# luo-yining/CFDBench

Hardware: NVIDIA H100
Metric: fno_rollout_steps_per_sec (higher is better)
Workload: dtype bf16

## Files before the change

### cfdbench_b200/_lib.py

```python
from __future__ import annotations

import ctypes as C
import os

_HERE = os.path.dirname(os.path.abspath(__file__))
LIB_PATH = os.path.join(_HERE, "libcfdbench_b200.so")

FNO_MAX_LAYERS = 8
ABI_VERSION = 4
ACT_F32, ACT_BF16 = 0, 1
EPI_GELU, EPI_GELU_SAVE_PRE, EPI_MUL_DGELU, EPI_PLAIN = 0, 1, 2, 3


class FnoWeights(C.Structure):
    _fields_ = [
        ("n_layers", C.c_int32),
        ("n_case_params", C.c_int32),
        ("fc0_w", C.c_void_p),
        ("fc0_b", C.c_void_p),
        ("spec_wk", C.c_void_p * FNO_MAX_LAYERS),
        ("w0t", C.c_void_p * FNO_MAX_LAYERS),
        ("w0_b", C.c_void_p * FNO_MAX_LAYERS),
        ("fc1_w", C.c_void_p),
        ("fc1_b", C.c_void_p),
# ... 28 lines not shown
    _fields_ = [("act", C.c_void_p * (FNO_MAX_LAYERS + 1)), ("pre", C.c_void_p * FNO_MAX_LAYERS),
                ("xm", C.c_void_p * FNO_MAX_LAYERS)]


class FnoWeightsBwd(C.Structure):
    _fields_ = [("spec_wkT", C.c_void_p * FNO_MAX_LAYERS), ("w0", C.c_void_p * FNO_MAX_LAYERS)]


class FnoBwdScratch(C.Structure):
    _fields_ = [("d", C.c_void_p * 2), ("dz1", C.c_void_p), ("gm", C.c_void_p), ("gwk", C.c_void_p),
                ("partials", C.c_void_p)]


BWD_CHUNK = 32
ADAM_MAX_TENSORS = 32


class FnoAdamTensors(C.Structure):
    _fields_ = [("count", C.c_int32),
                ("param", C.c_void_p * ADAM_MAX_TENSORS), ("grad", C.c_void_p * ADAM_MAX_TENSORS),
                ("exp_avg", C.c_void_p * ADAM_MAX_TENSORS), ("exp_avg_sq", C.c_void_p * ADAM_MAX_TENSORS),
                ("n", C.c_int64 * ADAM_MAX_TENSORS)]


class FnoNoise(C.Structure):
    _fields_ = [("std", C.c_float), ("seed", C.c_uint64), ("idx", C.c_void_p), ("step_base", C.c_void_p),
                ("step_offset", C.c_void_p), ("k0", C.c_int32)]


NOISE_STREAMS = 2 ** 16

_P = C.c_void_p
_I = C.c_int
_F = C.c_float

SIGNATURES = {
    "fno_version": (C.c_int, []),
    "fno_last_error": (C.c_char_p, []),
    "fno_destroy": (C.c_int, []),
    "fno_act_bytes": (C.c_size_t, [_I, _I]),
    "fno_modes_bytes": (C.c_size_t, [_I]),
    "fno_z_bytes": (C.c_size_t, [_I]),
    "fno_ym_image_bytes": (C.c_size_t, [_I]),
    "fno_bwd_partials_bytes": (C.c_size_t, []),
    "fno_mode_mix_image": (C.c_int, [_P, _P, _P, _I, _P]),
    "fno_block_fused": (C.c_int, [_P, _P, _P, _P, _P, _I, _P]),
    "fno_pack_spectral_weights": (C.c_int, [_P, _P, _P, _I, _P]),
    "fno_unpack_spectral_grads": (C.c_int, [_P, _P, _P, _P]),
    "fno_mix_operand_bytes": (C.c_size_t, []),
    "fno_pack_mix_operand": (C.c_int, [_P, _P, _P]),
    "fno_pack_mix_operand_from_weights": (C.c_int, [_P, _P, _P, _I, _P]),
    "fno_lift_fwd": (C.c_int, [_P, _P, _P, C.POINTER(FnoWeights), _P, _I, _I, _P]),
    "fno_spectral_dft_fwd": (C.c_int, [_P, _P, _I, _I, _F, _F, _P]),
    "fno_mode_mix": (C.c_int, [_P, _P, _P, _I, _P]),
    "fno_spectral_inv_kx": (C.c_int, [_P, _P, _I, _F, _F, _P]),
    "fno_block_out": (C.c_int, [_I, _P, _P, _P, _P, _P, _P, _P, _I, _I, _P]),
    "fno_block_fwd": (C.c_int, [C.POINTER(FnoWeights), _I, _P, _P, _P, C.POINTER(FnoWorkspace), _I, _I, _P]),
    "fno_project_fwd": (C.c_int, [_P, _P, C.POINTER(FnoWeights), _P, _I, _I, _P]),
    "fno_forward": (C.c_int, [C.POINTER(FnoWeights), _P, _P, _P, _P, C.POINTER(FnoWorkspace), _I, _I, _P]),
    "fno_rollout": (C.c_int, [C.POINTER(FnoWeights), _P, _P, _P, _P, _I, C.POINTER(FnoWorkspace), _I, _I, _P]),
    "fno_rollout_host": (C.c_int, [C.POINTER(FnoWeights), _P, _P, _P, _P, _I, C.POINTER(FnoWorkspace), _P, _I, _I, _P]),
    "fno_rollout_host_scratch_bytes": (C.c_size_t, [_I, _I, _I]),
    "fno_multistep_metrics": (C.c_int, [_P, _P, _P, _P, _I, _I, _P]),
    "fno_gather_batch": (C.c_int, [_P, _P, _P, _P, _P, _I, _I, _I, _P, _P, _P, _P, _P]),
    "fno_loss_scratch_bytes": (C.c_size_t, []),
    "fno_loss_fwd": (C.c_int, [_P, _P, C.c_size_t, _P, _P, _P]),
    "fno_loss_bwd": (C.c_int, [_P, _P, _P, _P, _P, C.c_size_t, _P]),
    "fno_adam_step": (C.c_int, [C.POINTER(FnoAdamTensors), C.c_float, C.c_float, C.c_float, C.c_float, C.c_float,
                                C.c_int64, _P]),
    "fno_train_stage_indices": (C.c_int, [_P, C.c_int64, _I, _I, _P, _P, _P]),
    "fno_adam_step_dev": (C.c_int, [C.POINTER(FnoAdamTensors), _P, _I, _P, _F, _F, _F, _F, _P]),
    "fno_adam_coefficients": (C.c_int, [_F, _F, _F, C.c_int64, _I, _P]),
    "fno_train_log_step": (C.c_int, [_P, _P, _I, _P, _P]),
    "fno_forward_train": (C.c_int, [C.POINTER(FnoWeights), _P, _P, _P, _P, C.POINTER(FnoTrainSaved),
                                    C.POINTER(FnoWorkspace), _I, _I, _P]),
    "fno_backward": (C.c_int, [C.POINTER(FnoWeights), C.POINTER(FnoWeightsBwd), _P, _P, _P, _P,
                               C.POINTER(FnoTrainSaved), C.POINTER(FnoGrads), C.POINTER(FnoBwdScratch),
                               C.POINTER(FnoWorkspace), _I, _I, _P]),
    "fno_backward_inputs": (C.c_int, [C.POINTER(FnoWeights), C.POINTER(FnoWeightsBwd), _P, _P, _P, _P,
                                      C.POINTER(FnoTrainSaved), C.POINTER(FnoGrads), C.POINTER(FnoBwdScratch),
                                      C.POINTER(FnoWorkspace), _P, _P, _I, _I, _P]),
    "fno_rollout_forward_train": (C.c_int, [C.POINTER(FnoWeights), _P, _P, _P, _P, _I, C.POINTER(FnoTrainSaved),
                                            C.POINTER(FnoWorkspace), _I, _I, _P]),
    "fno_rollout_backward": (C.c_int, [C.POINTER(FnoWeights), C.POINTER(FnoWeightsBwd), _P, _P, _P, _P, _P, _I,
                                       C.POINTER(FnoTrainSaved), C.POINTER(FnoGrads), C.POINTER(FnoBwdScratch),
                                       C.POINTER(FnoWorkspace), _P, _P, _P, _I, _I, _P]),
    "fno_grid_act_bytes": (C.c_size_t, [_I, _I, _I]),
    "fno_grid_z_bytes": (C.c_size_t, [_I, _I]),
    "fno_grid_bwd_partials_bytes": (C.c_size_t, [_I, _I]),
    "fno_grid_lift_fwd": (C.c_int, [_P, _P, _P, C.POINTER(FnoWeights), _P, _I, _I, _I, _P]),
    "fno_grid_spectral_dft_fwd": (C.c_int, [_P, _P, _I, _I, _I, _F, _F, _P]),
    "fno_grid_spectral_inv_kx": (C.c_int, [_P, _P, _I, _I, _I, _F, _F, _P]),
    "fno_grid_block_out": (C.c_int, [_I, _P, _P, _P, _P, _P, _P, _P, _I, _I, _I, _P]),
    "fno_grid_project_fwd": (C.c_int, [_P, _P, C.POINTER(FnoWeights), _P, _I, _I, _I, _P]),
    "fno_grid_project_bwd": (C.c_int, [_P, _P, _P, _P, C.POINTER(FnoWeights), _P, _P, _P, _P, _P, _P, _P, _I, _I, _I, _P]),
    "fno_grid_forward": (C.c_int, [C.POINTER(FnoWeights), _P, _P, _P, _P, C.POINTER(FnoWorkspace), _I, _I, _I, _P]),
    "fno_grid_rollout": (C.c_int, [C.POINTER(FnoWeights), _P, _P, _P, _P, _I, C.POINTER(FnoWorkspace), _I, _I, _I, _P]),
    "fno_grid_forward_train": (C.c_int, [C.POINTER(FnoWeights), _P, _P, _P, _P, C.POINTER(FnoTrainSaved),
                                         C.POINTER(FnoWorkspace), _I, _I, _I, _P]),
    "fno_grid_backward": (C.c_int, [C.POINTER(FnoWeights), C.POINTER(FnoWeightsBwd), _P, _P, _P, _P,
                                    C.POINTER(FnoTrainSaved), C.POINTER(FnoGrads), C.POINTER(FnoBwdScratch),
                                    C.POINTER(FnoWorkspace), _P, _P, _I, _I, _I, _P]),
    "fno_grid_rollout_forward_train": (C.c_int, [C.POINTER(FnoWeights), _P, _P, _P, _P, _I, C.POINTER(FnoTrainSaved),
                                                 C.POINTER(FnoWorkspace), _I, _I, _I, _P]),
    "fno_grid_rollout_backward": (C.c_int, [C.POINTER(FnoWeights), C.POINTER(FnoWeightsBwd), _P, _P, _P, _P, _P, _I,
                                            C.POINTER(FnoTrainSaved), C.POINTER(FnoGrads), C.POINTER(FnoBwdScratch),
# ... 65 lines not shown
```

### cfdbench_b200/csrc/fno_abi.cu

```cuda
#include <stdio.h>
#include <string.h>

#include "../../include/cfdbench_b200.h"
#include "fno_common.cuh"

namespace fno {
cudaError_t launch_dft_fwd(const void*, void*, int, float, float, cudaStream_t);
cudaError_t launch_mode_mix(const void*, const void*, void*, void*, int, cudaStream_t);
cudaError_t launch_block_fused(const void*, const void*, const float*, const float*, void*, int, cudaStream_t);
size_t ym_image_bytes(int);
cudaError_t launch_pack_spectral(const void*, const void*, void*, int, cudaStream_t);
cudaError_t launch_unpack_spectral(const void*, void*, void*, int, cudaStream_t);
cudaError_t launch_dft_fwd_tc(const void*, void*, int, float, float, cudaStream_t);
cudaError_t launch_pack_mix_operand(const void*, void*, cudaStream_t);
cudaError_t launch_pack_mix_operand_direct(const void*, const void*, void*, int, cudaStream_t);
size_t mix_operand_bytes();
cudaError_t launch_gather_batch(const void*, const void*, const float*, const int*, const long long*, int, int, int, float*,
                                float*, float*, float*, cudaStream_t);
cudaError_t launch_loss_fwd(const float*, const float*, size_t, float*, float*, cudaStream_t);
cudaError_t launch_loss_bwd(const float*, const float*, const float*, const float*, float*, size_t, cudaStream_t);
size_t loss_scratch_bytes();
cudaError_t launch_adam_step(const fno_adam_tensors*, float, float, float, float, float, long long, cudaStream_t);
cudaError_t launch_adam_step_dev(const fno_adam_tensors*, const float*, int, const int*, float, float, float, float,
                                 cudaStream_t);
void adam_coefficients(float, float, float, long long, float*, float*);
cudaError_t launch_stage_indices(const long long*, long long, int, int, const int*, long long*, cudaStream_t);
cudaError_t launch_log_step(const float*, float*, int, int*, cudaStream_t);
cudaError_t launch_inv_kx(const void*, void*, int, float, float, cudaStream_t);
template <typename TAct>
cudaError_t launch_block_tc(int, const void*, const void*, const float*, const float*, void*, float*, const float*, int,
                            cudaStream_t);
template <typename TAct>
cudaError_t launch_lift(const float*, const float*, const float*, const float*, const float*, const float*,
                        const float*, void*, int, int, cudaStream_t);
template <typename TAct>
cudaError_t launch_project_tc(const void*, const float*, const float*, const float*, const float*, const float*,
                              float*, int, cudaStream_t);
int project_bwd_rows_max();
int project_bwd_row();
cudaError_t launch_reduce_partials(const float*, int, int, float*, int, float*, int, float*, int, int, cudaStream_t);
template <typename TAct>
cudaError_t launch_project_bwd_tc(const void*, const float*, const float*, const float*, const float*, const float*, const float*,
                                  float*, float*, float*, int*, int, cudaStream_t);
template <typename TP, typename TQ, int NJ, int NI>
cudaError_t launch_chan_outer(const void*, const void*, float*, int*, int, cudaStream_t);
cudaError_t launch_multistep_metrics(const float*, const float*, const float*, float*, int, int, cudaStream_t);
cudaError_t launch_spectral_wgrad(const void*, const void*, void*, int, cudaStream_t);
cudaError_t launch_lift_bwd(const float*, const float*, const float*, const float*, const float*, const float*,
                            float*, float*, float*, int, int, int, cudaStream_t);
cudaError_t launch_lift_bwd_data(const float*, const float*, float*, float*, const float*, int, int, int, cudaStream_t);
bool grid_ok(int, int);
void grid_tables_release(int);
cudaError_t launch_grid_lift(const float*, const float*, const float*, const float*, const float*, const float*,
                             const float*, float*, int, int, int, int, cudaStream_t);
cudaError_t launch_grid_dft(const float*, void*, int, int, int, float, float, cudaStream_t);
cudaError_t launch_grid_inv_kx(const void*, float*, int, int, int, float, float, cudaStream_t);
cudaError_t launch_grid_block_out(int, const float*, const float*, const float*, const float*, float*, float*, const float*,
                                  int, int, int, cudaStream_t);
cudaError_t launch_grid_project(const float*, const float*, const float*, const float*, const float*, const float*, float*,
                                int, int, cudaStream_t);
cudaError_t launch_grid_project_bwd(const float*, const float*, const float*, const float*, const float*, const float*,
                                    const float*, float*, float*, float*, int, int, cudaStream_t);
int grid_project_bwd_parts(int, int);
int grid_project_bwd_row();
template <int NJ, int NI>
cudaError_t launch_grid_chan_outer(const float*, const float*, float*, int*, int, int, cudaStream_t);
// ... 135 lines not shown
const char* fno_last_error(void) { return g_err; }

size_t fno_act_bytes(int batch, int act_dtype) {
  return static_cast<size_t>(batch) * kC * kHW * (act_dtype == FNO_ACT_BF16 ? 2 : 4);
}
size_t fno_modes_bytes(int batch) { return static_cast<size_t>(batch) * kModes * kC * sizeof(float2); }
size_t fno_z_bytes(int batch) { return static_cast<size_t>(batch) * kH * 2 * kM2 * kC * sizeof(float); }
size_t fno_ym_image_bytes(int batch) { return ym_image_bytes(batch); }
size_t fno_bwd_partials_bytes(void) {
  return (static_cast<size_t>(296) * (kProj * kC + kProj) + static_cast<size_t>(project_bwd_rows_max()) * project_bwd_row() +
          static_cast<size_t>(16) * kC * (5 + kMaxCaseParams + 1)) * sizeof(float);
}

int fno_pack_spectral_weights(const void* w1, const void* w2, void* wk, int conj_transpose, void* stream) {
  if (!w1 || !w2 || !wk) return fail(kErrArg, "fno_pack_spectral_weights: null pointer");
  FNO_CUDA(launch_pack_spectral(w1, w2, wk, conj_transpose, S(stream)), "pack_spectral_kernel");
  return kOk;
}

size_t fno_mix_operand_bytes(void) { return mix_operand_bytes(); }

int fno_pack_mix_operand(const void* wk, void* wop, void* stream) {
  if (!wk || !wop) return fail(kErrArg, "fno_pack_mix_operand: null pointer");
  FNO_CUDA(launch_pack_mix_operand(wk, wop, S(stream)), "pack_mix_operand_kernel");
  return kOk;
}

int fno_pack_mix_operand_from_weights(const void* w1, const void* w2, void* wop, int conj_transpose, void* stream) {
  if (!w1 || !w2 || !wop) return fail(kErrArg, "fno_pack_mix_operand_from_weights: null pointer");
  FNO_CUDA(launch_pack_mix_operand_direct(w1, w2, wop, conj_transpose, S(stream)), "pack_mix_operand_direct_kernel");
  return kOk;
}

int fno_unpack_spectral_grads(const void* gwk, void* gw1, void* gw2, void* stream) {
  if (!gwk || !gw1 || !gw2) return fail(kErrArg, "fno_unpack_spectral_grads: null pointer");
  FNO_CUDA(launch_unpack_spectral(gwk, gw1, gw2, 0, S(stream)), "unpack_spectral_kernel");
  return kOk;
}

int fno_lift_fwd(const float* inputs, const float* mask, const float* case_params, const fno_weights* w,
                 void* act_out, int batch, int act_dtype, void* stream) {
  if (!inputs || !mask || !w || !act_out || batch <= 0 || bad_dtype(act_dtype))
    return fail(kErrArg, "fno_lift_fwd: bad argument");
  if (w->n_case_params > 0 && !case_params) return fail(kErrArg, "fno_lift_fwd: case_params is null");
  cudaError_t e = act_dtype == FNO_ACT_F32
                      ? launch_lift<float>(inputs, mask, case_params, w->fc0_w, w->fc0_b, w->gx, w->gy, act_out, batch,
                                           w->n_case_params, S(stream))
                      : launch_lift<__nv_bfloat16>(inputs, mask, case_params, w->fc0_w, w->fc0_b, w->gx, w->gy,
                                                   act_out, batch, w->n_case_params, S(stream));
  FNO_CUDA(e, "lift_kernel");
  return kOk;
}

int fno_spectral_dft_fwd(const void* act_in, void* xm, int batch, int act_dtype, float s0, float s1, void* stream) {
  if (!act_in || !xm || batch <= 0 || bad_dtype(act_dtype)) return fail(kErrArg, "fno_spectral_dft_fwd: bad argument");
  if (act_dtype == FNO_ACT_BF16) {
    FNO_CUDA(launch_dft_fwd_tc(act_in, xm, batch, s0, s1, S(stream)), "dft_fwd_tc_kernel");
    return kOk;
  }
  FNO_CUDA(launch_dft_fwd(act_in, xm, batch, s0, s1, S(stream)), "dft_fwd_kernel");
  return kOk;
}

int fno_mode_mix(const void* xm, const void* wk, void* ym, int batch, void* stream) {
  if (!xm || !wk || !ym || batch <= 0) return fail(kErrArg, "fno_mode_mix: bad argument");
  FNO_CUDA(launch_mode_mix(xm, wk, ym, nullptr, batch, S(stream)), "mode_mix_tc_kernel");
  return kOk;
}

int fno_mode_mix_image(const void* xm, const void* wk, void* ym_img, int batch, void* stream) {
  if (!xm || !wk || !ym_img || batch <= 0) return fail(kErrArg, "fno_mode_mix_image: bad argument");
  FNO_CUDA(launch_mode_mix(xm, wk, nullptr, ym_img, batch, S(stream)), "mode_mix_tc_kernel(image)");
  return kOk;
}

int fno_block_fused(const void* ym_img, const void* act_in, const float* w0t, const float* bias, void* act_out, int batch,
                    void* stream) {
  if (!ym_img || !act_in || !w0t || !act_out || batch <= 0) return fail(kErrArg, "fno_block_fused: bad argument");
  FNO_CUDA(launch_block_fused(ym_img, act_in, w0t, bias, act_out, batch, S(stream)), "block_fused_kernel");
  return kOk;
}

int fno_spectral_inv_kx(const void* ym, void* z, int batch, float s0, float s1, void* stream) {
  if (!ym || !z || batch <= 0) return fail(kErrArg, "fno_spectral_inv_kx: bad argument");
  FNO_CUDA(launch_inv_kx(ym, z, batch, s0, s1, S(stream)), "inv_kx_kernel");
  return kOk;
}

int fno_block_out(int epilogue, const void* z, const void* act_in, const float* w0t, const float* bias, void* act_out,
                  float* pre_out, const float* pre_in, int batch, int act_dtype, void* stream) {
  if (!z || !act_in || !w0t || !act_out || batch <= 0 || bad_dtype(act_dtype))
    return fail(kErrArg, "fno_block_out: bad argument");
  if (epilogue == FNO_EPI_GELU_SAVE_PRE && !pre_out) return fail(kErrArg, "fno_block_out: pre_out is null");
  if (epilogue == FNO_EPI_MUL_DGELU && !pre_in) return fail(kErrArg, "fno_block_out: pre_in is null");
  cudaError_t e = act_dtype == FNO_ACT_F32
                      ? launch_block_tc<float>(epilogue, z, act_in, w0t, bias, act_out, pre_out, pre_in, batch, S(stream))
                      : launch_block_tc<__nv_bfloat16>(epilogue, z, act_in, w0t, bias, act_out, pre_out, pre_in, batch,
                                                       S(stream));
  FNO_CUDA(e, "block_tc_kernel");
  return kOk;
}

int fno_block_fwd(const fno_weights* w, int layer, const void* act_in, void* act_out, float* pre_out,
                  const fno_workspace* ws, int batch, int act_dtype, void* stream) {
  if (!w || !ws || layer < 0 || layer >= w->n_layers) return fail(kErrArg, "fno_block_fwd: bad argument");
  FNO_TRY(fno_spectral_dft_fwd(act_in, ws->xm, batch, act_dtype, 1.f, 1.f, stream));
  if (act_dtype == FNO_ACT_BF16 && ws->ym_img && !pre_out) {
    FNO_TRY(fno_mode_mix_image(ws->xm, w->spec_wk[layer], ws->ym_img, batch, stream));
    return fno_block_fused(ws->ym_img, act_in, w->w0t[layer], w->w0_b[layer], act_out, batch, stream);
  }
  FNO_TRY(fno_mode_mix(ws->xm, w->spec_wk[layer], ws->ym, batch, stream));
  const float inv = 1.f / static_cast<float>(kHW);
  FNO_TRY(fno_spectral_inv_kx(ws->ym, ws->z, batch, inv, 2.f * inv, stream));
  return fno_block_out(pre_out ? FNO_EPI_GELU_SAVE_PRE : FNO_EPI_GELU, ws->z, act_in, w->w0t[layer], w->w0_b[layer],
                       act_out, pre_out, nullptr, batch, act_dtype, stream);
}

int fno_project_fwd(const void* act_in, const float* mask, const fno_weights* w, float* preds, int batch,
                    int act_dtype, void* stream) {
  if (!act_in || !mask || !w || !preds || batch <= 0 || bad_dtype(act_dtype))
    return fail(kErrArg, "fno_project_fwd: bad argument");
  cudaError_t e =
      act_dtype == FNO_ACT_F32
          ? launch_project_tc<float>(act_in, w->fc1_w, w->fc1_b, w->fc2_w, w->fc2_b, mask, preds, batch, S(stream))
          : launch_project_tc<__nv_bfloat16>(act_in, w->fc1_w, w->fc1_b, w->fc2_w, w->fc2_b, mask, preds, batch, S(stream));
  FNO_CUDA(e, "project_kernel");
  return kOk;
}

int fno_forward(const fno_weights* w, const float* inputs, const float* mask, const float* case_params,
                float* preds, const fno_workspace* ws, int batch, int act_dtype, void* stream) {
  if (!w || !ws || !ws->act[0] || !ws->act[1] || !ws->xm) return fail(kErrArg, "fno_forward: bad workspace");
  if (!(act_dtype == FNO_ACT_BF16 && ws->ym_img) && (!ws->ym || !ws->z)) return fail(kErrArg, "fno_forward: bad workspace");
  if (w->n_layers < 1 || w->n_layers > FNO_MAX_LAYERS) return fail(kErrUnsupported, "fno_forward: n_layers out of range");
  FNO_TRY(fno_lift_fwd(inputs, mask, case_params, w, ws->act[0], batch, act_dtype, stream));
  int cur = 0;
  for (int l = 0; l < w->n_layers; ++l) {
    FNO_TRY(fno_block_fwd(w, l, ws->act[cur], ws->act[cur ^ 1], nullptr, ws, batch, act_dtype, stream));
    cur ^= 1;
  }
  return fno_project_fwd(ws->act[cur], mask, w, preds, batch, act_dtype, stream);
}

static int rollout_impl(const char* what, const fno_weights* w, const float* inputs, const float* mask,
                        const float* case_params, float* preds_seq, int steps, const fno_workspace* ws, const fno_noise* nz,
                        float* fed, int batch, int act_dtype, void* stream) {
  char msg[160];
  if (steps < 0 || !preds_seq) {
    snprintf(msg, sizeof(msg), "%s: bad argument", what);
    return fail(kErrArg, msg);
  }
  const size_t frame = static_cast<size_t>(batch) * 2 * kHW;
  const float* cur = inputs;
  for (int s = 0; s < steps; ++s) {
    float* nxt = preds_seq + static_cast<size_t>(s) * frame;
    FNO_TRY(feed_step(nz, fed, mask, s, frame, batch, kH, kW, cur, stream));
    FNO_TRY(fno_forward(w, cur, mask, case_params, nxt, ws, batch, act_dtype, stream));
    cur = nxt;
  }
  return kOk;
}

int fno_rollout(const fno_weights* w, const float* inputs, const float* mask, const float* case_params,
                float* preds_seq, int steps, const fno_workspace* ws, int batch, int act_dtype, void* stream) {
  return rollout_impl("fno_rollout", w, inputs, mask, case_params, preds_seq, steps, ws, nullptr, nullptr, batch, act_dtype,
                      stream);
}

int fno_rollout_noise(const fno_weights* w, const float* inputs, const float* mask, const float* case_params,
                      float* preds_seq, int steps, const fno_workspace* ws, const fno_noise* noise, float* fed, int batch,
                      int act_dtype, void* stream) {
  FNO_TRY(noise_args("fno_rollout_noise", noise, fed, steps));
  FNO_TRY(noise_forward_args("fno_rollout_noise", w, inputs, mask, case_params, nullptr, ws, batch, false, act_dtype));
  return rollout_impl("fno_rollout_noise", w, inputs, mask, case_params, preds_seq, steps, ws, noise, fed, batch, act_dtype,
                      stream);
}

size_t fno_rollout_host_scratch_bytes(int batch, int n_case_params, int steps) {
  const size_t b = static_cast<size_t>(batch);
  return (b * 2 * kHW + b * kHW + static_cast<size_t>(steps) * b * 2 * kHW) * sizeof(float) +
         ((b * n_case_params * sizeof(float) + 255) / 256) * 256;
}

int fno_rollout_host(const fno_weights* w, const float* inputs_host, const float* mask_host,
                     const float* case_params_host, float* preds_seq_host, int steps, const fno_workspace* ws,
                     void* dev_io, int batch, int act_dtype, void* stream) {
  if (!w || !inputs_host || !mask_host || !preds_seq_host || !dev_io || batch <= 0 || steps <= 0)
    return fail(kErrArg, "fno_rollout_host: bad argument");
  const size_t b = static_cast<size_t>(batch);
  float* d_in = static_cast<float*>(dev_io);
  float* d_mask = d_in + b * 2 * kHW;
  float* d_seq = d_mask + b * kHW;
  float* d_params = d_seq + static_cast<size_t>(steps) * b * 2 * kHW;
  cudaStream_t st = S(stream);
  FNO_CUDA(cudaMemcpyAsync(d_in, inputs_host, b * 2 * kHW * sizeof(float), cudaMemcpyHostToDevice, st), "H2D inputs");
  FNO_CUDA(cudaMemcpyAsync(d_mask, mask_host, b * kHW * sizeof(float), cudaMemcpyHostToDevice, st), "H2D mask");
  if (w->n_case_params > 0)
    FNO_CUDA(cudaMemcpyAsync(d_params, case_params_host, b * w->n_case_params * sizeof(float), cudaMemcpyHostToDevice, st),
             "H2D case_params");
  FNO_TRY(fno_rollout(w, d_in, d_mask, d_params, d_seq, steps, ws, batch, act_dtype, stream));
  FNO_CUDA(cudaMemcpyAsync(preds_seq_host, d_seq, static_cast<size_t>(steps) * b * 2 * kHW * sizeof(float),
                           cudaMemcpyDeviceToHost, st),
           "D2H preds");
  return kOk;
}

static int forward_train_body(const fno_weights* w, const float* inputs, const float* mask, const float* case_params,
                              const fno_train_saved* saved, const fno_workspace* ws, int batch, int act_dtype, void* stream) {
  FNO_TRY(fno_lift_fwd(inputs, mask, case_params, w, saved->act[0], batch, act_dtype, stream));
  const float inv = 1.f / static_cast<float>(kHW);
  for (int l = 0; l < w->n_layers; ++l) {
    if (!saved->act[l + 1] || !saved->pre[l] || !saved->xm[l]) return fail(kErrArg, "fno_forward_train: null saved buffer");
    FNO_TRY(fno_spectral_dft_fwd(saved->act[l], saved->xm[l], batch, act_dtype, 1.f, 1.f, stream));
    FNO_TRY(fno_mode_mix(saved->xm[l], w->spec_wk[l], ws->ym, batch, stream));
    FNO_TRY(fno_spectral_inv_kx(ws->ym, ws->z, batch, inv, 2.f * inv, stream));
    FNO_TRY(fno_block_out(FNO_EPI_GELU_SAVE_PRE, ws->z, saved->act[l], w->w0t[l], w->w0_b[l], saved->act[l + 1],
                          saved->pre[l], nullptr, batch, act_dtype, stream));
  }
  return kOk;
}

int fno_forward_train(const fno_weights* w, const float* inputs, const float* mask, const float* case_params,
                      float* preds, const fno_train_saved* saved, const fno_workspace* ws, int batch,
                      int act_dtype, void* stream) {
  if (!w || !saved || !ws || !ws->ym || !ws->z) return fail(kErrArg, "fno_forward_train: bad argument");
  if (w->n_layers < 1 || w->n_layers > FNO_MAX_LAYERS) return fail(kErrUnsupported, "fno_forward_train: n_layers");
  FNO_TRY(forward_train_body(w, inputs, mask, case_params, saved, ws, batch, act_dtype, stream));
  return fno_project_fwd(saved->act[w->n_layers], mask, w, preds, batch, act_dtype, stream);
}

static int backward_impl(const char* what, const fno_weights* w, const fno_weights_bwd* wb, const float* inputs,
                         const float* mask, const float* case_params, const float* dpreds, const fno_train_saved* saved,
                         const fno_grads* g, const fno_bwd_scratch* sc, const fno_workspace* ws, int batch, int act_dtype,
                         void* stream, float* d_inputs, float* d_case_params, int accum = 0, int hand_off = 0,
                         const float* add = nullptr) {
  char msg[128];
  if (!w || !wb || !inputs || !mask || !dpreds || !saved || !sc || !ws || batch <= 0 || bad_dtype(act_dtype)) {
    snprintf(msg, sizeof(msg), "%s: bad argument", what);
    return fail(kErrArg, msg);
  }
  if (!sc->d[0] || !sc->d[1] || !sc->dz1 || !sc->gm || !sc->gwk || !sc->partials || !ws->ym || !ws->z) {
    snprintf(msg, sizeof(msg), "%s: null scratch buffer", what);
    return fail(kErrArg, msg);
  }
  cudaStream_t st = S(stream);
  const int L = w->n_layers, p = w->n_case_params;
  const bool bf = act_dtype == FNO_ACT_BF16;
  float* part_co = sc->partials;
  float* part_pb = part_co + static_cast<size_t>(296) * (kProj * kC + kProj);
  float* part_lb = part_pb + static_cast<size_t>(project_bwd_rows_max()) * project_bwd_row();
  const size_t act_elt = bf ? 2 : 4;
  for (int b0 = 0; b0 < batch; b0 += FNO_BWD_CHUNK) {
    const int nb = (batch - b0 < FNO_BWD_CHUNK) ? batch - b0 : FNO_BWD_CHUNK;
    const char* a_l = static_cast<const char*>(saved->act[L]) + static_cast<size_t>(b0) * kC * kHW * act_elt;
    const float* pre = saved->pre[L - 1] + static_cast<size_t>(b0) * kC * kHW;
    float* dout = sc->d[0] + static_cast<size_t>(b0) * kC * kHW;
    const float* dp = dpreds + static_cast<size_t>(b0) * 2 * kHW;
    const float* mk = mask + static_cast<size_t>(b0) * kHW;
    int rows = 0;
    cudaError_t e =
        bf ? launch_project_bwd_tc<__nv_bfloat16>(a_l, dp, mk, pre, w->fc1_w, w->fc1_b, w->fc2_w, dout, sc->dz1, part_pb, &rows, nb, st)
           : launch_project_bwd_tc<float>(a_l, dp, mk, pre, w->fc1_w, w->fc1_b, w->fc2_w, dout, sc->dz1, part_pb, &rows, nb, st);
    FNO_CUDA(e, "project_bwd_tc_kernel");
    if (!g) continue;
    const int acc_c = (accum || b0 > 0) ? 1 : 0;
    FNO_CUDA(launch_reduce_partials(part_pb, rows, project_bwd_row(), g->fc2_w, 2 * kProj, g->fc1_b, kProj, g->fc2_b, 2, acc_c, st),
// ... 785 lines not shown
```

### cfdbench_b200/csrc/fno_dft_fwd_tc.cu

```cuda
#include "fno_common.cuh"
#include "tc_common.cuh"
#include "tc_tma.cuh"
#include <math.h>
#include <stddef.h>
#include <string.h>

namespace fno {

constexpr int kTdWG = 2;
constexpr int kTdThreads = 128 * kTdWG;
constexpr int kTdPlanes = 8;
constexpr int kTdBoxPlanes = 2;
constexpr int kTdBoxes = kTdPlanes / kTdBoxPlanes;
constexpr int kTdSlots = 3;
constexpr uint32_t kTdPlaneBytes = kHW * 2;
constexpr uint32_t kTdBoxBytes = kTdBoxPlanes * kTdPlaneBytes;
constexpr int kTdNA = 72;
constexpr uint32_t kTdLboTA = (kTdNA / 8) * 128;
constexpr uint32_t kTdTABytes = 8 * kTdLboTA;
constexpr int kTdM2 = kM2 * 2 * kTdPlanes;
constexpr int kTdN2 = 2 * kKX;
constexpr int kTdK2 = kH;
constexpr uint32_t kTdLboT = (kTdN2 / 8) * 128;
constexpr int kTdTFloats = kTdN2 * kTdK2;
// ... 81 lines not shown
      if (t == 0 && n + kTdSlots < n_fills) load(n + kTdSlots);
      if (k == 0) tc::named_barrier(1 + wg, 128);
#pragma unroll
      for (int p = 0; p < kTdBoxPlanes; ++p)
#pragma unroll
        for (int g3 = 0; g3 < 3; ++g3)
#pragma unroll
          for (int hh = 0; hh < 2; ++hh)
#pragma unroll
            for (int ri = 0; ri < 2; ++ri) {
              const int c = 4 * (3 * g3) + 2 * hh + ri;
              g[td_g_index(16 * (4 * g3 + q) + 8 * ri + kTdBoxPlanes * k + p, m0 + 8 * hh)] =
                  (ga[p][c + 8] + ga[p][c + 4]) + ga[p][c];
            }
    }
    tc::named_barrier(1 + wg, 128);
    const int unit = td_unit(first, stride, i);
    const int b = unit * kTdPlanes / kC, c0 = unit * kTdPlanes % kC;
#pragma unroll 1
    for (int tile = 0; tile < kTdM2 / 64; ++tile) {
      uint32_t a_hi[kTdK2 / 8][4], a_lo[kTdK2 / 8][4];
#pragma unroll
      for (int ks = 0; ks < kTdK2 / 8; ++ks)
#pragma unroll
        for (int r = 0; r < 4; ++r) {
          float hi, lo;
          tc::split_tf32(g[td_g_index(64 * tile + m0 + 8 * (r & 1), 8 * ks + q + 4 * (r >> 1))], hi, lo);
          a_hi[ks][r] = __float_as_uint(hi);
          a_lo[ks][r] = __float_as_uint(lo);
        }
      float d[24];
      tc::wg_fence();
#pragma unroll
      for (int pass = 0; pass < 3; ++pass) {
        const uint32_t tb = tc::smem_addr(pass == 1 ? sm.t_lo : sm.t_hi);
#pragma unroll
        for (int ks = 0; ks < kTdK2 / 8; ++ks)
          tc::wg_tf32_rs_n48(d, pass == 2 ? a_lo[ks] : a_hi[ks], tc::make_smem_desc(tb + ks * 2 * kTdLboT, kTdLboT, 128),
                             (pass | ks) ? 1u : 0u);
      }
      tc::wg_commit();
      tc::wg_wait<0>();
      tc::wg_fence_acc(d);
      const int qq = 4 * tile + wq;
      const float sc = qq == 0 ? s0 : s1;
#pragma unroll
      for (int j = 0; j < kTdN2 / 8; ++j) {
        const int kxi = 4 * j + q;
        const float re = (d[4 * j + 0] + d[4 * j + 3]) * sc, im = (d[4 * j + 2] - d[4 * j + 1]) * sc;
        xm[(static_cast<size_t>(kxi * kM2 + qq) * batch + b) * kC + c0 + lr] = make_float2(re, im);
      }
    }
  }
}

static uint16_t td_bf16_bits(double v) {
  float f = static_cast<float>(v);
  uint32_t u;
  memcpy(&u, &f, 4);
  const uint32_t r = u + 0x7fffu + ((u >> 16) & 1u);
  return static_cast<uint16_t>(r >> 16);
}
static double td_bf16_value(uint16_t b) {
  const uint32_t u = static_cast<uint32_t>(b) << 16;
  float f;
  memcpy(&f, &u, 4);
  return static_cast<double>(f);
}
static float td_round_tf32(double v) {
  float f = static_cast<float>(v);
  uint32_t u;
  memcpy(&u, &f, 4);
  u = (u + 0x1000u) & 0xffffe000u;
  memcpy(&f, &u, 4);
  return f;
}

struct TdTables {
  unsigned char* ta = nullptr;
  float* t = nullptr;
  int n_sm = 0;
  bool configured = false;
};
static TdTables g_td[64];

static cudaError_t td_ensure(int dev, cudaStream_t stream) {
  TdTables& t = g_td[dev];
  if (t.configured) return cudaSuccess;
  static unsigned char h_ta[kTdTABytes];
  static float h_t[2 * kTdTFloats];
  memset(h_ta, 0, sizeof(h_ta));
  memset(h_t, 0, sizeof(h_t));
  const double two_pi = 2.0 * 3.14159265358979323846;
  for (int q = 0; q < kM2; ++q)
    for (int ri = 0; ri < 2; ++ri)
      for (int w = 0; w < 64; ++w) {
        const double ang = two_pi * ((q * w) % 64) / 64.0;
        double rest = ri ? -sin(ang) : cos(ang);
        for (int t3 = 0; t3 < 3; ++t3) {
          const int row = 8 * (3 * (q >> 2) + t3) + 2 * (q & 3) + ri;
          const size_t off = static_cast<size_t>(w >> 3) * kTdLboTA + (row >> 3) * 128 + (row & 7) * 16 + (w & 7) * 2;
          const uint16_t bits = td_bf16_bits(rest);
          memcpy(h_ta + off, &bits, 2);
          rest -= td_bf16_value(bits);
        }
      }
  for (int kxi = 0; kxi < kKX; ++kxi) {
    const int kx = kxi < kM1 ? kxi : kxi + (kH - kKX);
    for (int cs = 0; cs < 2; ++cs)
      for (int h = 0; h < kH; ++h) {
        const double ang = two_pi * ((kx * h) % 64) / 64.0;
        const double val = cs ? sin(ang) : cos(ang);
        const uint32_t off = tc::kmajor_offset(2 * kxi + cs, h, kTdN2) / 4;
        const float hi = td_round_tf32(val);
        h_t[off] = hi;
        h_t[kTdTFloats + off] = td_round_tf32(val - static_cast<double>(hi));
      }
  }
  cudaError_t e = cudaMalloc(&t.ta, sizeof(h_ta));
  if (e != cudaSuccess) return e;
  e = cudaMalloc(&t.t, sizeof(h_t));
  if (e != cudaSuccess) return e;
  e = cudaMemcpyAsync(t.ta, h_ta, sizeof(h_ta), cudaMemcpyHostToDevice, stream);
  if (e != cudaSuccess) return e;
  e = cudaMemcpyAsync(t.t, h_t, sizeof(h_t), cudaMemcpyHostToDevice, stream);
  if (e != cudaSuccess) return e;
  e = cudaStreamSynchronize(stream);
  if (e != cudaSuccess) return e;
  e = cudaFuncSetAttribute(dft_fwd_tc_kernel, cudaFuncAttributeMaxDynamicSharedMemorySize, (int)sizeof(TdSmem));
  if (e != cudaSuccess) return e;
  e = cudaDeviceGetAttribute(&t.n_sm, cudaDevAttrMultiProcessorCount, dev);
  if (e != cudaSuccess) return e;
  t.configured = true;
  return cudaSuccess;
}

void dft_fwd_tc_release(int dev) {
  if (dev < 0 || dev >= 64) return;
  TdTables& t = g_td[dev];
  if (t.ta) cudaFree(t.ta);
  if (t.t) cudaFree(t.t);
  t = TdTables();
}

cudaError_t launch_dft_fwd_tc(const void* x, void* xm, int batch, float s0, float s1, cudaStream_t stream) {
  int dev = 0;
  cudaError_t e = cudaGetDevice(&dev);
  if (e != cudaSuccess) return e;
  if (dev < 0 || dev >= 64) return cudaErrorInvalidDevice;
  e = td_ensure(dev, stream);
  if (e != cudaSuccess) return e;
  if ((reinterpret_cast<uintptr_t>(x) & 15) || (reinterpret_cast<uintptr_t>(xm) & 15)) return cudaErrorMisalignedAddress;
  CUtensorMap map;
  e = make_tma_map_2d(&map, CU_TENSOR_MAP_DATA_TYPE_BFLOAT16, 2, x, kW, static_cast<uint64_t>(batch) * kC * kH, kW,
                      kTdBoxPlanes * kH);
  if (e != cudaSuccess) return e;
  const int n_units = batch * kC / kTdPlanes;
  const int per_pipe = (n_units + kTdWG * g_td[dev].n_sm - 1) / (kTdWG * g_td[dev].n_sm);
  const int grid = (n_units + kTdWG * per_pipe - 1) / (kTdWG * per_pipe);
  return launch_chained(dft_fwd_tc_kernel, dim3(grid), dim3(kTdThreads), sizeof(TdSmem), stream, map,
                        static_cast<float2*>(xm), static_cast<const unsigned char*>(g_td[dev].ta),
                        static_cast<const float*>(g_td[dev].t), n_units, batch, s0, s1);
}

}
```

### include/cfdbench_b200.h

```cpp
#ifndef CFDBENCH_B200_H_
#define CFDBENCH_B200_H_

#include <stddef.h>
#include <stdint.h>

#ifdef __cplusplus
extern "C" {
#endif

#define FNO_ABI_VERSION 4
#define FNO_MAX_LAYERS 8

enum { FNO_ACT_F32 = 0, FNO_ACT_BF16 = 1 };
enum { FNO_EPI_GELU = 0, FNO_EPI_GELU_SAVE_PRE = 1, FNO_EPI_MUL_DGELU = 2, FNO_EPI_PLAIN = 3 };

typedef struct fno_weights {
  int32_t n_layers;
  int32_t n_case_params;
  const float* fc0_w;
  const float* fc0_b;
  const void* spec_wk[FNO_MAX_LAYERS];
  const float* w0t[FNO_MAX_LAYERS];
  const float* w0_b[FNO_MAX_LAYERS];
  const float* fc1_w;
  const float* fc1_b;
  const float* fc2_w;
  const float* fc2_b;
  const float* gx;
  const float* gy;
} fno_weights;

typedef struct fno_workspace {
  void* act[2];
  void* xm;
  void* ym;
  void* z;
  void* ym_img;
} fno_workspace;

int fno_version(void);
int fno_destroy(void);
const char* fno_last_error(void);
size_t fno_act_bytes(int batch, int act_dtype);
size_t fno_modes_bytes(int batch);
size_t fno_z_bytes(int batch);
size_t fno_ym_image_bytes(int batch);
size_t fno_bwd_partials_bytes(void);

int fno_pack_spectral_weights(const void* weights1, const void* weights2, void* wk, int conj_transpose, void* stream);
size_t fno_mix_operand_bytes(void);
int fno_pack_mix_operand(const void* wk, void* wop, void* stream);
int fno_pack_mix_operand_from_weights(const void* weights1, const void* weights2, void* wop, int conj_transpose,
                                      void* stream);
int fno_unpack_spectral_grads(const void* gwk, void* gw1, void* gw2, void* stream);

int fno_lift_fwd(const float* inputs, const float* mask, const float* case_params, const fno_weights* w,
                 void* act_out, int batch, int act_dtype, void* stream);

int fno_spectral_dft_fwd(const void* act_in, void* xm, int batch, int act_dtype, float s0, float s1, void* stream);
int fno_mode_mix(const void* xm, const void* wop, void* ym, int batch, void* stream);
int fno_spectral_inv_kx(const void* ym, void* z, int batch, float s0, float s1, void* stream);
int fno_block_out(int epilogue, const void* z, const void* act_in, const float* w0t, const float* bias, void* act_out,
                  float* pre_out, const float* pre_in, int batch, int act_dtype, void* stream);
int fno_mode_mix_image(const void* xm, const void* wop, void* ym_img, int batch, void* stream);
int fno_block_fused(const void* ym_img, const void* act_in_bf16, const float* w0t, const float* bias, void* act_out_bf16,
                    int batch, void* stream);
int fno_block_fwd(const fno_weights* w, int layer, const void* act_in, void* act_out, float* pre_out,
                  const fno_workspace* ws, int batch, int act_dtype, void* stream);

int fno_project_fwd(const void* act_in, const float* mask, const fno_weights* w, float* preds, int batch,
                    int act_dtype, void* stream);

int fno_forward(const fno_weights* w, const float* inputs, const float* mask, const float* case_params,
                float* preds, const fno_workspace* ws, int batch, int act_dtype, void* stream);

int fno_rollout(const fno_weights* w, const float* inputs, const float* mask, const float* case_params,
                float* preds_seq, int steps, const fno_workspace* ws, int batch, int act_dtype, void* stream);

int fno_rollout_host(const fno_weights* w, const float* inputs_host, const float* mask_host,
                     const float* case_params_host, float* preds_seq_host, int steps, const fno_workspace* ws,
                     void* dev_io, int batch, int act_dtype, void* stream);
size_t fno_rollout_host_scratch_bytes(int batch, int n_case_params, int steps);


typedef struct fno_train_saved {
  void* act[FNO_MAX_LAYERS + 1];
  float* pre[FNO_MAX_LAYERS];
  void* xm[FNO_MAX_LAYERS];
} fno_train_saved;

typedef struct fno_weights_bwd {
  const void* spec_wkT[FNO_MAX_LAYERS];
  const float* w0[FNO_MAX_LAYERS];
} fno_weights_bwd;

typedef struct fno_grads {
  float* fc0_w;
  float* fc0_b;
  void* spec_w1[FNO_MAX_LAYERS];
  void* spec_w2[FNO_MAX_LAYERS];
  float* w0_w[FNO_MAX_LAYERS];
  float* w0_b[FNO_MAX_LAYERS];
  float* fc1_w;
  float* fc1_b;
  float* fc2_w;
  float* fc2_b;
} fno_grads;

typedef struct fno_bwd_scratch {
  float* d[2];
// ... 171 lines not shown
```

Before: 1362.

## Fuse lift projection with first-layer forward DFT in one kernel

Adds a kernel that computes the lifted bf16 activation in shared memory and immediately runs the tensor-core forward DFT on it, writing the activation out via TMA stores while the spectral modes are produced. The first block then starts from the precomputed modes, which removes one kernel launch and the re-read of the lifted activation from global memory. The cost is a larger, more complex kernel with heavy shared-memory use and a new code path limited to bf16.

Result: faster. 1383, median of 6 (+1.5%).

```diff
diff --git a/cfdbench_b200/_lib.py b/cfdbench_b200/_lib.py
--- a/cfdbench_b200/_lib.py
+++ b/cfdbench_b200/_lib.py
@@ -104,6 +104,7 @@
     "fno_pack_mix_operand_from_weights": (C.c_int, [_P, _P, _P, _I, _P]),
     "fno_lift_fwd": (C.c_int, [_P, _P, _P, C.POINTER(FnoWeights), _P, _I, _I, _P]),
     "fno_spectral_dft_fwd": (C.c_int, [_P, _P, _I, _I, _F, _F, _P]),
+    "fno_lift_dft_fwd": (C.c_int, [_P, _P, _P, C.POINTER(FnoWeights), _P, _P, _I, _P]),
     "fno_mode_mix": (C.c_int, [_P, _P, _P, _I, _P]),
     "fno_spectral_inv_kx": (C.c_int, [_P, _P, _I, _F, _F, _P]),
     "fno_block_out": (C.c_int, [_I, _P, _P, _P, _P, _P, _P, _P, _I, _I, _P]),
diff --git a/cfdbench_b200/csrc/fno_abi.cu b/cfdbench_b200/csrc/fno_abi.cu
--- a/cfdbench_b200/csrc/fno_abi.cu
+++ b/cfdbench_b200/csrc/fno_abi.cu
@@ -12,6 +12,8 @@
 cudaError_t launch_pack_spectral(const void*, const void*, void*, int, cudaStream_t);
 cudaError_t launch_unpack_spectral(const void*, void*, void*, int, cudaStream_t);
 cudaError_t launch_dft_fwd_tc(const void*, void*, int, float, float, cudaStream_t);
+cudaError_t launch_lift_dft_fwd_tc(const float*, const float*, const float*, const float*, const float*, const float*,
+                                   const float*, void*, void*, int, int, cudaStream_t);
 cudaError_t launch_pack_mix_operand(const void*, void*, cudaStream_t);
 cudaError_t launch_pack_mix_operand_direct(const void*, const void*, void*, int, cudaStream_t);
 size_t mix_operand_bytes();
@@ -253,6 +255,16 @@
   return kOk;
 }
 
+int fno_lift_dft_fwd(const float* inputs, const float* mask, const float* case_params, const fno_weights* w,
+                     void* act_out, void* xm, int batch, void* stream) {
+  if (!inputs || !mask || !w || !act_out || !xm || batch <= 0) return fail(kErrArg, "fno_lift_dft_fwd: bad argument");
+  if (w->n_case_params > 0 && !case_params) return fail(kErrArg, "fno_lift_dft_fwd: case_params is null");
+  FNO_CUDA(launch_lift_dft_fwd_tc(inputs, mask, case_params, w->fc0_w, w->fc0_b, w->gx, w->gy, act_out, xm, batch,
+                                  w->n_case_params, S(stream)),
+           "lift_dft_fwd_tc_kernel");
+  return kOk;
+}
+
 int fno_spectral_dft_fwd(const void* act_in, void* xm, int batch, int act_dtype, float s0, float s1, void* stream) {
   if (!act_in || !xm || batch <= 0 || bad_dtype(act_dtype)) return fail(kErrArg, "fno_spectral_dft_fwd: bad argument");
   if (act_dtype == FNO_ACT_BF16) {
@@ -302,10 +314,10 @@
   return kOk;
 }
 
-int fno_block_fwd(const fno_weights* w, int layer, const void* act_in, void* act_out, float* pre_out,
-                  const fno_workspace* ws, int batch, int act_dtype, void* stream) {
-  if (!w || !ws || layer < 0 || layer >= w->n_layers) return fail(kErrArg, "fno_block_fwd: bad argument");
-  FNO_TRY(fno_spectral_dft_fwd(act_in, ws->xm, batch, act_dtype, 1.f, 1.f, stream));
+}
+
+static int block_fwd_from_modes(const fno_weights* w, int layer, const void* act_in, void* act_out, float* pre_out,
+                                const fno_workspace* ws, int batch, int act_dtype, void* stream) {
   if (act_dtype == FNO_ACT_BF16 && ws->ym_img && !pre_out) {
     FNO_TRY(fno_mode_mix_image(ws->xm, w->spec_wk[layer], ws->ym_img, batch, stream));
     return fno_block_fused(ws->ym_img, act_in, w->w0t[layer], w->w0_b[layer], act_out, batch, stream);
@@ -315,6 +327,15 @@
   FNO_TRY(fno_spectral_inv_kx(ws->ym, ws->z, batch, inv, 2.f * inv, stream));
   return fno_block_out(pre_out ? FNO_EPI_GELU_SAVE_PRE : FNO_EPI_GELU, ws->z, act_in, w->w0t[layer], w->w0_b[layer],
                        act_out, pre_out, nullptr, batch, act_dtype, stream);
+}
+
+extern "C" {
+
+int fno_block_fwd(const fno_weights* w, int layer, const void* act_in, void* act_out, float* pre_out,
+                  const fno_workspace* ws, int batch, int act_dtype, void* stream) {
+  if (!w || !ws || layer < 0 || layer >= w->n_layers) return fail(kErrArg, "fno_block_fwd: bad argument");
+  FNO_TRY(fno_spectral_dft_fwd(act_in, ws->xm, batch, act_dtype, 1.f, 1.f, stream));
+  return block_fwd_from_modes(w, layer, act_in, act_out, pre_out, ws, batch, act_dtype, stream);
 }
 
 int fno_project_fwd(const void* act_in, const float* mask, const fno_weights* w, float* preds, int batch,
@@ -334,9 +355,15 @@
   if (!w || !ws || !ws->act[0] || !ws->act[1] || !ws->xm) return fail(kErrArg, "fno_forward: bad workspace");
   if (!(act_dtype == FNO_ACT_BF16 && ws->ym_img) && (!ws->ym || !ws->z)) return fail(kErrArg, "fno_forward: bad workspace");
   if (w->n_layers < 1 || w->n_layers > FNO_MAX_LAYERS) return fail(kErrUnsupported, "fno_forward: n_layers out of range");
-  FNO_TRY(fno_lift_fwd(inputs, mask, case_params, w, ws->act[0], batch, act_dtype, stream));
-  int cur = 0;
-  for (int l = 0; l < w->n_layers; ++l) {
+  if (act_dtype == FNO_ACT_BF16) {
+    FNO_TRY(fno_lift_dft_fwd(inputs, mask, case_params, w, ws->act[0], ws->xm, batch, stream));
+    FNO_TRY(block_fwd_from_modes(w, 0, ws->act[0], ws->act[1], nullptr, ws, batch, act_dtype, stream));
+  } else {
+    FNO_TRY(fno_lift_fwd(inputs, mask, case_params, w, ws->act[0], batch, act_dtype, stream));
+    FNO_TRY(fno_block_fwd(w, 0, ws->act[0], ws->act[1], nullptr, ws, batch, act_dtype, stream));
+  }
+  int cur = 1;
+  for (int l = 1; l < w->n_layers; ++l) {
     FNO_TRY(fno_block_fwd(w, l, ws->act[cur], ws->act[cur ^ 1], nullptr, ws, batch, act_dtype, stream));
     cur ^= 1;
   }
@@ -408,11 +435,16 @@
 
 static int forward_train_body(const fno_weights* w, const float* inputs, const float* mask, const float* case_params,
                               const fno_train_saved* saved, const fno_workspace* ws, int batch, int act_dtype, void* stream) {
-  FNO_TRY(fno_lift_fwd(inputs, mask, case_params, w, saved->act[0], batch, act_dtype, stream));
+  if (!saved->act[0] || !saved->xm[0]) return fail(kErrArg, "fno_forward_train: null saved buffer");
+  if (act_dtype == FNO_ACT_BF16)
+    FNO_TRY(fno_lift_dft_fwd(inputs, mask, case_params, w, saved->act[0], saved->xm[0], batch, stream));
+  else
+    FNO_TRY(fno_lift_fwd(inputs, mask, case_params, w, saved->act[0], batch, act_dtype, stream));
   const float inv = 1.f / static_cast<float>(kHW);
   for (int l = 0; l < w->n_layers; ++l) {
     if (!saved->act[l + 1] || !saved->pre[l] || !saved->xm[l]) return fail(kErrArg, "fno_forward_train: null saved buffer");
-    FNO_TRY(fno_spectral_dft_fwd(saved->act[l], saved->xm[l], batch, act_dtype, 1.f, 1.f, stream));
+    if (l > 0 || act_dtype != FNO_ACT_BF16)
+      FNO_TRY(fno_spectral_dft_fwd(saved->act[l], saved->xm[l], batch, act_dtype, 1.f, 1.f, stream));
     FNO_TRY(fno_mode_mix(saved->xm[l], w->spec_wk[l], ws->ym, batch, stream));
     FNO_TRY(fno_spectral_inv_kx(ws->ym, ws->z, batch, inv, 2.f * inv, stream));
     FNO_TRY(fno_block_out(FNO_EPI_GELU_SAVE_PRE, ws->z, saved->act[l], w->w0t[l], w->w0_b[l], saved->act[l + 1],
diff --git a/cfdbench_b200/csrc/fno_dft_fwd_tc.cu b/cfdbench_b200/csrc/fno_dft_fwd_tc.cu
--- a/cfdbench_b200/csrc/fno_dft_fwd_tc.cu
+++ b/cfdbench_b200/csrc/fno_dft_fwd_tc.cu
@@ -157,6 +157,194 @@
       }
     }
   }
+}
+
+constexpr int kLdSlots = 3;
+constexpr int kLdBands = 4;
+constexpr int kLdBandRows = kH / kLdBands;
+constexpr uint32_t kLdSlotBytes = kTdPlanes * kLdBandRows * kW * 2;
+static_assert(kLdSlots >= 2 && kLdSlotBytes == 128u * 128u, "a slot is 128 swizzled lines of 128 bytes");
+
+__host__ __device__ constexpr int ld_slot(int n) { return n % kLdSlots; }
+__host__ __device__ constexpr int ld_box_h(int n) { return (n % kLdBands) * kLdBandRows; }
+__host__ __device__ constexpr int ld_box_plane(int unit) { return unit * kTdPlanes; }
+__host__ __device__ constexpr uint32_t ld_chunk_offset(int plane, int hb, int chunk) {
+  return static_cast<uint32_t>((plane * kLdBandRows + hb) * 128 + ((chunk ^ (hb & 7)) << 4));
+}
+
+struct LdSmem {
+  alignas(1024) unsigned char x[kTdWG][kLdSlots][kLdSlotBytes];
+  alignas(128) unsigned char ta[kTdTABytes];
+  alignas(128) float t_hi[kTdTFloats];
+  alignas(128) float t_lo[kTdTFloats];
+  alignas(128) float g[kTdWG][kTdM2 * kTdK2];
+  alignas(16) float4 lw[kTdWG][2][kTdPlanes][2];
+};
+static_assert(sizeof(LdSmem) <= 232448, "lift_dft_fwd_tc_kernel exceeds the sm_90 opt-in shared memory");
+
+__global__ void __launch_bounds__(kTdThreads, 1)
+    lift_dft_fwd_tc_kernel(const __grid_constant__ CUtensorMap a0_map, float2* __restrict__ xm,
+                           const unsigned char* __restrict__ ta_tab, const float* __restrict__ t_tab,
+                           const float* __restrict__ inputs, const float* __restrict__ mask,
+                           const float* __restrict__ params, const float* __restrict__ w, const float* __restrict__ bias,
+                           const float* __restrict__ gx, const float* __restrict__ gy, int p, int n_units, int batch) {
+  extern __shared__ __align__(1024) unsigned char smem_raw[];
+  LdSmem& sm = *reinterpret_cast<LdSmem*>(smem_raw);
+  if ((smem_u32(smem_raw) & 1023u) != 0) __trap();
+  const int tid = threadIdx.x, lane = tid & 31;
+  const int wg = tc::warp_index_uniform() >> 2, wq = (tid >> 5) & 3, t = tid & 127, q = lane & 3, lr = lane >> 2;
+  const int first = blockIdx.x * kTdWG + wg, stride = gridDim.x * kTdWG;
+  const int n_mine = td_units_of(first, stride, n_units);
+  const int n_fills = n_mine * kLdBands;
+  const int hb = t >> 3, chunk = t & 7;
+
+  for (int e = tid; e < static_cast<int>(kTdTABytes / 16); e += kTdThreads)
+    reinterpret_cast<uint4*>(sm.ta)[e] = __ldg(reinterpret_cast<const uint4*>(ta_tab) + e);
+  for (int e = tid; e < kTdTFloats / 4; e += kTdThreads) {
+    reinterpret_cast<float4*>(sm.t_hi)[e] = __ldg(reinterpret_cast<const float4*>(t_tab) + e);
+    reinterpret_cast<float4*>(sm.t_lo)[e] = __ldg(reinterpret_cast<const float4*>(t_tab + kTdTFloats) + e);
+  }
+  pdl_wait();
+  pdl_launch_dependents();
+
+  const int nin = 5 + p;
+  auto unit_consts = [&](int i) {
+    const int unit = td_unit(first, stride, i);
+    const int b = unit * kTdPlanes / kC, c = unit * kTdPlanes % kC + t;
+    float cb = bias[c];
+    for (int j = 0; j < p; ++j) cb = fmaf(w[c * nin + 5 + j], params[b * p + j], cb);
+    sm.lw[wg][i & 1][t][0] = make_float4(w[c * nin + 0], w[c * nin + 1], w[c * nin + 2], w[c * nin + 3]);
+    sm.lw[wg][i & 1][t][1] = make_float4(w[c * nin + 4], cb, 0.f, 0.f);
+  };
+  if (t < kTdPlanes && n_mine > 0) unit_consts(0);
+  float yw[8];
+  *reinterpret_cast<float4*>(yw) = *reinterpret_cast<const float4*>(gy + 8 * chunk);
+  *reinterpret_cast<float4*>(yw + 4) = *reinterpret_cast<const float4*>(gy + 8 * chunk + 4);
+  float4 fu[2][2], fv[2][2], fm[2][2];
+  float fx[2];
+  auto fetch = [&](int n, int s) {
+    const int unit = td_unit(first, stride, n / kLdBands);
+    const size_t b = static_cast<size_t>(unit * kTdPlanes / kC);
+    const int pix = (ld_box_h(n) + hb) * kW + 8 * chunk;
+    const float4* u4 = reinterpret_cast<const float4*>(inputs + (b * 2 + 0) * kHW + pix);
+    const float4* v4 = reinterpret_cast<const float4*>(inputs + (b * 2 + 1) * kHW + pix);
+    const float4* m4 = reinterpret_cast<const float4*>(mask + b * kHW + pix);
+    fu[s][0] = u4[0]; fu[s][1] = u4[1];
+    fv[s][0] = v4[0]; fv[s][1] = v4[1];
+    fm[s][0] = m4[0]; fm[s][1] = m4[1];
+    fx[s] = gx[ld_box_h(n) + hb];
+  };
+  static_assert(kLdBands % 2 == 0, "fill n's prefetch buffer is k % 2");
+  for (int n = 0; n < 2 && n < n_fills; ++n) fetch(n, n);
+  tc::fence_proxy_async_smem();
+  __syncthreads();
+
+  const int m0 = 16 * wq + lr;
+  const uint32_t ta_s = tc::smem_addr(sm.ta);
+  float* g = sm.g[wg];
+#pragma unroll 1
+  for (int i = 0; i < n_mine; ++i) {
+#pragma unroll
+    for (int k = 0; k < kLdBands; ++k) {
+      const int n = i * kLdBands + k;
+      unsigned char* slot = sm.x[wg][ld_slot(n)];
+      {
+        const float4* pu = fu[k & 1];
+        const float4* pv = fv[k & 1];
+        const float4* pm = fm[k & 1];
+        const float u[8] = {pu[0].x, pu[0].y, pu[0].z, pu[0].w, pu[1].x, pu[1].y, pu[1].z, pu[1].w};
+        const float v[8] = {pv[0].x, pv[0].y, pv[0].z, pv[0].w, pv[1].x, pv[1].y, pv[1].z, pv[1].w};
+        const float m[8] = {pm[0].x, pm[0].y, pm[0].z, pm[0].w, pm[1].x, pm[1].y, pm[1].z, pm[1].w};
+        const float xh = fx[k & 1];
+#pragma unroll
+        for (int pl = 0; pl < kTdPlanes; ++pl) {
+          const float4 w0 = sm.lw[wg][i & 1][pl][0], w1 = sm.lw[wg][i & 1][pl][1];
+          const float base = fmaf(w0.w, xh, w1.y);
+          float r[8];
+#pragma unroll
+          for (int j = 0; j < 8; ++j) r[j] = fmaf(w0.x, u[j], fmaf(w0.y, v[j], fmaf(w0.z, m[j], fmaf(w1.x, yw[j], base))));
+          uint4 pk;
+          __nv_bfloat162 h2;
+          h2 = __floats2bfloat162_rn(r[0], r[1]); pk.x = *reinterpret_cast<uint32_t*>(&h2);
+          h2 = __floats2bfloat162_rn(r[2], r[3]); pk.y = *reinterpret_cast<uint32_t*>(&h2);
+          h2 = __floats2bfloat162_rn(r[4], r[5]); pk.z = *reinterpret_cast<uint32_t*>(&h2);
+          h2 = __floats2bfloat162_rn(r[6], r[7]); pk.w = *reinterpret_cast<uint32_t*>(&h2);
+          *reinterpret_cast<uint4*>(slot + ld_chunk_offset(pl, hb, chunk)) = pk;
+        }
+      }
+      if (n + 2 < n_fills) fetch(n + 2, k & 1);
+      tc::fence_proxy_async_smem();
+      if (t == 0) bulk_wait_group_read<kLdSlots - 2>();
+      tc::named_barrier(1 + wg, 128);
+      if (t == 0) {
+        tma_store_3d(&a0_map, slot, 0, ld_box_h(n), ld_box_plane(td_unit(first, stride, i)));
+        bulk_commit_group();
+      }
+      float ga[2][36];
+      tc::wg_fence();
+      const uint32_t x_s = tc::smem_addr(slot);
+#pragma unroll
+      for (int j = 0; j < 2; ++j)
+#pragma unroll
+        for (int ks = 0; ks < kW / 16; ++ks)
+          tc::wg_bf16_ss_n72(ga[j], tc::make_smem_desc_sw128(x_s + j * (kLdSlotBytes / 2) + ks * 32),
+                             tc::make_smem_desc(ta_s + ks * 2 * kTdLboTA, kTdLboTA, 128), ks ? 1u : 0u);
+      tc::wg_commit();
+      if (k == 0 && t < kTdPlanes && i + 1 < n_mine) unit_consts(i + 1);
+      tc::wg_wait<0>();
+      tc::wg_fence_acc(ga[0]);
+      tc::wg_fence_acc(ga[1]);
+#pragma unroll
+      for (int j = 0; j < 2; ++j)
+#pragma unroll
+        for (int g3 = 0; g3 < 3; ++g3)
+#pragma unroll
+          for (int hh = 0; hh < 2; ++hh)
+#pragma unroll
+            for (int ri = 0; ri < 2; ++ri) {
+              const int c = 4 * (3 * g3) + 2 * hh + ri;
+              g[td_g_index(16 * (4 * g3 + q) + 8 * ri + 4 * j + wq, ld_box_h(n) + lr + 8 * hh)] =
+                  (ga[j][c + 8] + ga[j][c + 4]) + ga[j][c];
+            }
+    }
+    tc::named_barrier(1 + wg, 128);
+    const int unit = td_unit(first, stride, i);
+    const int b = unit * kTdPlanes / kC, c0 = unit * kTdPlanes % kC;
+#pragma unroll 1
+    for (int tile = 0; tile < kTdM2 / 64; ++tile) {
+      uint32_t a_hi[kTdK2 / 8][4], a_lo[kTdK2 / 8][4];
+#pragma unroll
+      for (int ks = 0; ks < kTdK2 / 8; ++ks)
+#pragma unroll
+        for (int r = 0; r < 4; ++r) {
+          float hi, lo;
+          tc::split_tf32(g[td_g_index(64 * tile + m0 + 8 * (r & 1), 8 * ks + q + 4 * (r >> 1))], hi, lo);
+          a_hi[ks][r] = __float_as_uint(hi);
+          a_lo[ks][r] = __float_as_uint(lo);
+        }
+      float d[24];
+      tc::wg_fence();
+#pragma unroll
+      for (int pass = 0; pass < 3; ++pass) {
+        const uint32_t tb = tc::smem_addr(pass == 1 ? sm.t_lo : sm.t_hi);
+#pragma unroll
+        for (int ks = 0; ks < kTdK2 / 8; ++ks)
+          tc::wg_tf32_rs_n48(d, pass == 2 ? a_lo[ks] : a_hi[ks], tc::make_smem_desc(tb + ks * 2 * kTdLboT, kTdLboT, 128),
+                             (pass | ks) ? 1u : 0u);
+      }
+      tc::wg_commit();
+      tc::wg_wait<0>();
+      tc::wg_fence_acc(d);
+      const int qq = 4 * tile + wq;
+#pragma unroll
+      for (int j = 0; j < kTdN2 / 8; ++j) {
+        const int kxi = 4 * j + q;
+        const float re = d[4 * j + 0] + d[4 * j + 3], im = d[4 * j + 2] - d[4 * j + 1];
+        xm[(static_cast<size_t>(kxi * kM2 + qq) * batch + b) * kC + c0 + lr] = make_float2(re, im);
+      }
+    }
+  }
+  if (t == 0) bulk_wait_group<0>();
 }
 
 static uint16_t td_bf16_bits(double v) {
@@ -234,6 +422,8 @@
   if (e != cudaSuccess) return e;
   e = cudaFuncSetAttribute(dft_fwd_tc_kernel, cudaFuncAttributeMaxDynamicSharedMemorySize, (int)sizeof(TdSmem));
   if (e != cudaSuccess) return e;
+  e = cudaFuncSetAttribute(lift_dft_fwd_tc_kernel, cudaFuncAttributeMaxDynamicSharedMemorySize, (int)sizeof(LdSmem));
+  if (e != cudaSuccess) return e;
   e = cudaDeviceGetAttribute(&t.n_sm, cudaDevAttrMultiProcessorCount, dev);
   if (e != cudaSuccess) return e;
   t.configured = true;
@@ -268,4 +458,29 @@
                         static_cast<const float*>(g_td[dev].t), n_units, batch, s0, s1);
 }
 
-}
+cudaError_t launch_lift_dft_fwd_tc(const float* inputs, const float* mask, const float* params, const float* w,
+                                   const float* bias, const float* gx, const float* gy, void* act, void* xm, int batch,
+                                   int p, cudaStream_t stream) {
+  if (p < 0 || p > kMaxCaseParams) return cudaErrorInvalidValue;
+  int dev = 0;
+  cudaError_t e = cudaGetDevice(&dev);
+  if (e != cudaSuccess) return e;
+  if (dev < 0 || dev >= 64) return cudaErrorInvalidDevice;
+  e = td_ensure(dev, stream);
+  if (e != cudaSuccess) return e;
+  for (const void* ptr : {static_cast<const void*>(inputs), static_cast<const void*>(mask), static_cast<const void*>(gy),
+                          static_cast<const void*>(act), static_cast<const void*>(xm)})
+    if (reinterpret_cast<uintptr_t>(ptr) & 15) return cudaErrorMisalignedAddress;
+  CUtensorMap map;
+  e = make_tma_map_3d(&map, CU_TENSOR_MAP_DATA_TYPE_BFLOAT16, 2, act, kW, kH, static_cast<uint64_t>(batch) * kC, kW,
+                      kLdBandRows, kTdPlanes);
+  if (e != cudaSuccess) return e;
+  const int n_units = batch * kC / kTdPlanes;
+  const int per_pipe = (n_units + kTdWG * g_td[dev].n_sm - 1) / (kTdWG * g_td[dev].n_sm);
+  const int grid = (n_units + kTdWG * per_pipe - 1) / (kTdWG * per_pipe);
+  return launch_chained(lift_dft_fwd_tc_kernel, dim3(grid), dim3(kTdThreads), sizeof(LdSmem), stream, map,
+                        static_cast<float2*>(xm), static_cast<const unsigned char*>(g_td[dev].ta),
+                        static_cast<const float*>(g_td[dev].t), inputs, mask, params, w, bias, gx, gy, p, n_units, batch);
+}
+
+}
diff --git a/include/cfdbench_b200.h b/include/cfdbench_b200.h
--- a/include/cfdbench_b200.h
+++ b/include/cfdbench_b200.h
@@ -56,6 +56,9 @@
 
 int fno_lift_fwd(const float* inputs, const float* mask, const float* case_params, const fno_weights* w,
                  void* act_out, int batch, int act_dtype, void* stream);
+
+int fno_lift_dft_fwd(const float* inputs, const float* mask, const float* case_params, const fno_weights* w,
+                     void* act_out_bf16, void* xm, int batch, void* stream);
 
 int fno_spectral_dft_fwd(const void* act_in, void* xm, int batch, int act_dtype, float s0, float s1, void* stream);
 int fno_mode_mix(const void* xm, const void* wop, void* ym, int batch, void* stream);
```
